# ztlpn/minilp

Hardware: AMD Instinct MI355X
Metric: simplex pivots/sec (higher is better)
Workload: dtype f64; 1 GPU; config 4: random LP 100000 vars x 100000 constraints, 100 nnz/row (0.1% fill), Max c'x, Ax<=b, x>=0; primal simplex with PSE+DSE from the slack basis; timed pivots 5..1983; parallelism=1 GPU, nucleus_size_at_end=1559, completed_steps=1978

## Files before the change

minilp_amd/csrc/engine.h:

```cpp
#pragma once
#include <hip/hip_runtime.h>

#include <cstdint>
#include <utility>
#include <stdexcept>
#include <string>
#include <vector>

#include "kernels.h"

namespace mlp {

enum Stage { STAGE_FTRAN = 0, STAGE_RATIO = 1, STAGE_BTRAN = 2, STAGE_BASIS = 3, STAGE_ROW = 4, STAGE_APPLY = 5 };

struct MlpError : std::runtime_error {
    int code;
    MlpError(int c, const std::string& s) : std::runtime_error(s), code(c) {}
};
struct LpFail {
    int code;
};

#define HIPCHECK(expr)                                                                                   \
    do {                                                                                                 \
// ... 285 lines not shown
    DevBuf<int> d_nb_order;
    DevBuf<int> d_pk_ptr;
    DevBuf<unsigned short> d_pk_row;
    DevBuf<double> d_pk_val;
    DevBuf<unsigned char> d_pk_valid;
    DevBuf<unsigned char> d_fmark;
    bool use_pack = true;
    bool pack_built = false;
    size_t band_total_ = 0;
    bool use_order = true;
    uint64_t order_built_at = 0;
    uint64_t lifetime_pivots = 0;
    uint64_t order_every = 2048;
    bool order_valid = false;
    uint64_t order_from = 4096;
    bool order_force = false;
    void refresh_nb_order(bool force);
    int det_mode = -1;
    int banded_mode = -1;
    bool use_banded() const;
  public:
    bool banded_active() const { return use_banded(); }
    bool factor_active() const { return fac_on_; }
    void restart_sampling() { batches_run = 0; }
  private:
    void ensure_banded();
    DevBuf<int> d_fpk_cnt, d_fpk_var;
    DevBuf<double> d_fpk_val, d_fpk_x, d_fpk_part;
    DevBuf<unsigned char> d_fpk_in;
    bool fpull_on_ = true;
    bool fpk_valid_ = false;
    uint64_t fpk_built_at_ = 0, fpk_builds_ = 0;
    int fpk_every_ = 1024;
    bool fpk_wanted() const;
    void fpk_rebuild();
    DevBuf<int> d_colblk;
    DevBuf<double> d_push_part;
    bool colblk_dirty = true;
    void ensure_colblk();
    DevBuf<double> d_sdiag_of_pos, d_W, d_U, d_V, d_Ut;
    int ld_pad = 16;
    int pad_for(int cap) const { return (cap >= 8192 || force_big_tiles) ? ld_pad : 0; }
    int ld() const { return cap_ + pad_for(cap_); }
    int lr_force = -1;
    DevBuf<double> d_work;
    DevBuf<double> d_alpha_r, d_helper;
    DevBuf<int2> d_nb_rng;
    int sweep_variant = 0;
    int sw_balanced = 1;
    int rt_device = 0;
    void acquire_runtime();
    void release_runtime();
    bool force_big_tiles = false;
    int shard_rank = 0, shard_world = 1;
    bool shard_defer_ = true;
    bool shard_live_ = false;
    bool shard_is_live() const { return shard_world > 1 && shard_live_; }
    MailRec* d_mail = nullptr;
    void* mail_host = nullptr;
    bool mail_registered = false;
    void* own_box = nullptr;
    void* peer_box[MAX_WORLD] = {};
    int mail_fanout = 1;
    size_t xb_cap_ = 0;
    bool no_wshard = false;
    void release_mailboxes();
    int pump_backend_ = 0;
// ... 106 lines not shown
```

minilp_amd/csrc/engine.hip:

```cpp
#include "engine.h"


#include <algorithm>
#include <chrono>
#include <cmath>
#include <cstdio>
#include <cstdlib>
#include <climits>
#include <cstring>
#include <limits>
#include <map>
#include <memory>
#include <mutex>

#include <dlfcn.h>
#include <fcntl.h>
#include <sys/mman.h>
#include <sys/stat.h>
#include <unistd.h>

namespace mlp {

static const double INF = std::numeric_limits<double>::infinity();
static double now_s() {
// ... 49 lines not shown
    force_big_tiles = bt && std::atoi(bt) != 0;
    const char* dm = std::getenv("MLP_DETERMINISTIC");
    if (dm) det_mode = std::atoi(dm) != 0 ? 1 : 0;
    const char* bd = std::getenv("MLP_BANDED");
    if (bd) banded_mode = std::atoi(bd) != 0 ? 1 : 0;
    const char* fr = std::getenv("MLP_FINAL_REFRESH");
    if (fr) final_refresh_pivots = std::atol(fr);
    if (const char* sp = std::getenv("MLP_SWEEP_PACKED")) use_pack = sp[0] != '0';
    if (const char* of = std::getenv("MLP_ORDER_FROM")) order_from = (uint64_t)std::atoll(of);
    if (const char* oe = std::getenv("MLP_ORDER_EVERY")) order_every = (uint64_t)std::atoll(oe);
    const char* lz = std::getenv("MLP_LAZY_DSE");
    lazy_dse = !(lz && lz[0] == '0');
    ratio_two = std::getenv("MLP_RATIO_TWO_KERNELS") != nullptr;
    if (const char* hy = std::getenv("MLP_HYPER")) hyper_mode = std::atoi(hy) > 0 ? 1 : 0;
    if (const char* phk = std::getenv("MLP_PRIMAL_HEAD_K")) ph_kmax = std::max(0, std::atoi(phk));
    if (const char* sbk = std::getenv("MLP_SMALL_BASIS_K")) sb_kmax = std::max(0, std::min(256, std::atoi(sbk)));
    if (const char* sk = std::getenv("MLP_STR_K")) str_kmax = std::atoi(sk);
    if (const char* hh = std::getenv("MLP_HYPER_HEAVY")) hyper_heavy = std::atol(hh);
    if (const char* rs = std::getenv("MLP_RATIO_SPIN_LIMIT")) ratio_spin_limit = std::atoll(rs);
    if (const char* sb = std::getenv("MLP_STREAM_BALANCED")) sw_balanced = std::atoi(sb);
    if (const char* fm = std::getenv("MLP_FACTOR")) fac_mode = std::atoi(fm) > 0 ? 1 : 0;
    if (const char* fj = std::getenv("MLP_FACTOR_J")) {
        fac_J_ = fac_period_ = std::max(1, std::min(64, std::atoi(fj)));
        fac_period_auto_ = false;
    }
    if (const char* ff = std::getenv("MLP_FACTOR_FROM")) fac_auto_cap_ = std::max(256, std::atoi(ff));
    if (const char* fb = std::getenv("MLP_FACTOR_BUMP")) {
        const int want = std::atoi(fb);
        fac_bump_max_ = std::max(0, std::min(FAC_BMAX, want));
        if (want < FAC_BMAX) fac_sb_max_ = std::min(fac_sb_max_, fac_bump_max_);
    }
    if (const char* fb = std::getenv("MLP_FACTOR_SB")) fac_sb_max_ = std::max(0, std::min(FAC_SB_MAX, std::atoi(fb)));
    if (const char* fb = std::getenv("MLP_FACTOR_SB_FROM")) fac_sb_from_ = std::max(1, std::atoi(fb));
    if (const char* fp = std::getenv("MLP_FPULL")) fpull_on_ = fp[0] != '0';
    const char* nws = std::getenv("MLP_NO_WSHARD");
    no_wshard = nws && std::atoi(nws) != 0;
    const char* bs = std::getenv("MLP_BATCH");
    if (bs) batch = std::max(1, std::min(RING, std::atoi(bs)));
    const char* gi = std::getenv("MLP_GRAPH_ITERS");
    if (gi) graph_iters = std::max(1, std::min(32, std::atoi(gi)));
}
namespace {
struct RtBundle {
    int device = 0;
    hipStream_t st = nullptr, st2 = nullptr;
    hipEvent_t evFork[3] = {nullptr, nullptr, nullptr}, evJoin[3] = {nullptr, nullptr, nullptr};
    Ctl* h_ctl = nullptr;
};
struct RtPool {
    std::mutex mu;
    std::vector<RtBundle> idle;
};
RtPool& rt_pool() {
    static RtPool* p = new RtPool();
    return *p;
}
constexpr size_t kMaxIdleRuntimes = 64;
}
void Engine::acquire_runtime() {
    int dev = 0;
    HIPCHECK(hipGetDevice(&dev));
    rt_device = dev;
    {
        RtPool& p = rt_pool();
        std::lock_guard<std::mutex> lk(p.mu);
        for (size_t i = 0; i < p.idle.size(); ++i)
            if (p.idle[i].device == dev) {
// ... 224 lines not shown
                d_pk_row.ensure(band_total_ + 16, 0, st);
                d_pk_val.ensure(band_total_ + 16, 0, st);
                if (d_pk_row.p != r0) HIPCHECK(hipMemsetAsync(d_pk_row.p, 0, sizeof(unsigned short) * d_pk_row.cap, st));
                if (d_pk_val.p != v0) HIPCHECK(hipMemsetAsync(d_pk_val.p, 0, sizeof(double) * d_pk_val.cap, st));
            }
            d_pk_valid.ensure((size_t)num_vars, 0, st);
            d_scan_tmp.ensure(np / 4096 + 8, 0, st);
        } catch (MlpError&) {
            (void)hipGetLastError();
            use_pack = false;
            return;
        }
        DevView t{};
        t.m = m_; t.n = num_vars; t.nbands = nb;
        t.bptr = d_bptr.p; t.brow = d_brow.p; t.bval = d_bval.p;
        t.nb_vars = d_nb_vars.p; t.nb_order = d_nb_order.p;
        launch_pack_count(t, d_pk_ptr.p, st);
        launch_exclusive_scan(d_pk_ptr.p, d_pk_ptr.p, (long)np, d_scan_tmp.p, st);
        launch_pack_fill(t, d_pk_ptr.p, d_pk_row.p, d_pk_val.p, d_pk_valid.p, st);
        HIPCHECK(hipStreamSynchronize(st));
        pack_built = true;
    }
}

void Engine::ensure_colblk() {
    if (!colblk_dirty) return;
    const int rb = (m_ + PB_ROWS - 1) / PB_ROWS;
    d_colblk.ensure((size_t)N_ * (rb + 1), 0, st);
    launch_build_colblk(d_cptr.p, d_crow.p, N_, rb, d_colblk.p, st);
    d_push_part.ensure((size_t)PB_CHUNKS * (size_t)m_, 0, st);
    colblk_dirty = false;
}

bool Engine::fpk_wanted() const {
    const int lr = fac_on_ ? 0 : (lr_force >= 0 ? lr_force : (cap_ >= 8192 ? 32 : 0));
    return fpull_on_ && !fac_on_ && !stepping && lr > 0 && enable_pse && d_rowinfo.p != nullptr;
}
void Engine::fpk_rebuild() {
    const size_t nnz = h_rcol.size();
    d_fpk_cnt.ensure((size_t)m_ + 8, 0, st);
    d_fpk_var.ensure(nnz + 8, 0, st);
    d_fpk_val.ensure(nnz + 8, 0, st);
    d_fpk_in.ensure((size_t)N_ + 8, 0, st);
    d_fpk_x.ensure((size_t)N_ + 8, 0, st);
    d_fpk_part.ensure(2 * (((size_t)m_ * 2 + 2048) / 32 + 8), 0, st);
    DevView t = *sync_view();
    t.fpk_cnt = d_fpk_cnt.p; t.fpk_var = d_fpk_var.p; t.fpk_val = d_fpk_val.p; t.fpk_in = d_fpk_in.p; t.fpk_x = d_fpk_x.p;
    HIPCHECK(hipMemsetAsync(d_fpk_in.p, 0, (size_t)N_, st));
    HIPCHECK(hipMemsetAsync(d_fpk_x.p, 0, sizeof(double) * (size_t)N_, st));
    launch_fpk_build(t, st);
    fpk_valid_ = true;
    fpk_built_at_ = lifetime_pivots;
    fpk_builds_ += 1;
    if (!hview.fpk_on || hview.fpk_cnt != d_fpk_cnt.p || hview.fpk_var != d_fpk_var.p || hview.fpk_val != d_fpk_val.p ||
        hview.fpk_in != d_fpk_in.p || hview.fpk_x != d_fpk_x.p || hview.fpk_part != d_fpk_part.p) {
        view_dirty = true;
        sync_view();
    }
}

DevView* Engine::sync_view() {
    if (!view_dirty) return &hview;
    DevView old = hview;
    DevView& v = hview;
    v.m = m_; v.n = num_vars; v.ld = ld(); v.pad0 = 0;
    v.csc_ptr = d_cptr.p; v.csc_row = d_crow.p; v.csc_val = d_cval.p;
    v.csr_ptr = d_rptr.p; v.csr_col = d_rcol.p; v.csr_val = d_rval.p;
    v.var_lo = d_lo.p; v.var_hi = d_hi.p; v.obj_c = d_obj.p;
    v.var_loc = d_var_loc.p;
    v.basic_vars = d_basic_vars.p; v.xB = d_xB.p; v.loB = d_loB.p; v.hiB = d_hiB.p; v.beta = d_beta.p;
    v.nb_vars = d_nb_vars.p; v.d = d_d.p; v.xN = d_xN.p; v.gamma = d_gamma.p; v.nbflags = d_nbflags.p;
    v.kslot_of_pos = d_kslot_of_pos.p; v.srow_of_pos = d_srow_of_pos.p; v.sdiag_of_pos = d_sdiag_of_pos.p;
    v.kslot_of_row = d_kslot_of_row.p; v.pos_of_srow = d_pos_of_srow.p; v.rowinfo = d_rowinfo.p;
    const bool shard_det = shard_world > 1;
    static const int pb_det_env = std::getenv("MLP_PB_DET") ? std::atoi(std::getenv("MLP_PB_DET")) : -1;
    int hbits = 1;
    while (hbits < 31 && (1 << hbits) <= max_row_nnz_) hbits += 1;
    const bool det_fits = hbits <= 20;
    const bool pb_det = det_fits && (shard_det || force_det_push_ || pb_det_env == 1 || (pb_det_env < 0 && pb_det_default));
    const bool pb_size = cap_ > 4096 || force_big_tiles ||
                         (shard_det && pb_det && cap_ >= 512 && det_mode != 1 && h_rcol.size() > ((size_t)1 << 21));
    v.pb_on = (pb_size && (!shard_det || pb_det)) ? 1 : 0;
    v.pb_det = (v.pb_on && pb_det) ? 1 : 0;
    v.pb_hbits = hbits;
    v.pb_amax = amax_;
    if (v.pb_on) ensure_colblk();
    v.colblk = v.pb_on ? d_colblk.p : nullptr;
    v.push_part = v.pb_on ? d_push_part.p : nullptr;
    v.pb_rb = (m_ + PB_ROWS - 1) / PB_ROWS;
    {
        if (!(fpk_wanted() && v.pb_on && (!v.pb_det || shard_world > 1))) fpk_valid_ = false;
        const bool fp = fpk_valid_ && d_fpk_cnt.p != nullptr;
        v.fpk_cnt = d_fpk_cnt.p; v.fpk_var = d_fpk_var.p; v.fpk_val = d_fpk_val.p; v.fpk_in = d_fpk_in.p;
        v.fpk_x = fp ? d_fpk_x.p : nullptr; v.fpk_part = d_fpk_part.p;
        v.fpk_on = fp ? 1 : 0; v.pad5 = 0;
    }
    v.det_pull = (!v.pb_on && (det_mode == 1 || shard_det || force_det_push_ || (det_mode < 0 && h_rcol.size() <= ((size_t)1 << 21)))) ? 1 : 0;
    if (v.det_pull) {
        const unsigned char* before = d_fmark.p;
        d_fmark.ensure((size_t)m_ + 64, 0, st);
        if (d_fmark.p != before) HIPCHECK(hipMemsetAsync(d_fmark.p, 0, d_fmark.cap, st));
        v.fmark = d_fmark.p;
    } else {
        v.fmark = nullptr;
    }
    v.banded = use_banded() ? 1 : 0;
    if (v.banded) ensure_banded();
    v.bptr = v.banded ? d_bptr.p : nullptr;
    v.brow = v.banded ? d_brow.p : nullptr;
    v.bval = v.banded ? d_bval.p : nullptr;
    v.band_part = v.banded ? d_band_part.p : nullptr;
    v.nbands = (m_ + BAND_ROWS - 1) / BAND_ROWS;
    if (v.banded && use_order && shard_world == 1 && (lifetime_pivots >= order_from || order_force)) {
        if (!order_valid || (use_pack && !pack_built)) refresh_nb_order(true);
        v.nb_order = d_nb_order.p;
    } else {
        v.nb_order = nullptr;
    }
    const bool pk = v.nb_order && use_pack && pack_built;
    v.pk_ptr = pk ? d_pk_ptr.p : nullptr; v.pk_row = pk ? d_pk_row.p : nullptr; v.pk_val = pk ? d_pk_val.p : nullptr;
    v.pk_valid = pk ? d_pk_valid.p : nullptr;
    v.pos_of_kslot = d_pos_of_kslot.p; v.row_of_kslot = d_row_of_kslot.p; v.W = d_W.p;
    v.U = d_U.p; v.V = d_V.p; v.Ut = d_Ut.p;
    v.lrJ = fac_on_ ? 0 : (lr_force >= 0 ? lr_force : (cap_ >= 8192 ? 32 : 0));
// ... 798 lines not shown
}
void Engine::get_values(double* out, int n) {
    fetch_values();
    for (int v = 0; v < n; ++v) {
        int loc = h_var_loc[v];
        out[v] = loc >= 0 ? h_xB[loc] : h_xN[-1 - loc];
    }
}
double Engine::cur_obj_val() {
    pull_ctl();
    return h_ctl->it.obj;
}

static const int kStageOrder[2][6] = {{STAGE_FTRAN, STAGE_RATIO, STAGE_BTRAN, STAGE_BASIS, STAGE_ROW, STAGE_APPLY},
                                      {STAGE_BTRAN, STAGE_ROW, STAGE_RATIO, STAGE_FTRAN, STAGE_BASIS, STAGE_APPLY}};
void Engine::launch_stage(int phase, int stage, bool with_events) {
    const DevView& dv = hview;
    const Geom g = geom();
    const int pse = enable_pse ? 1 : 0;
    const bool lazy = lazy_now(phase);
    const int dse = (enable_dse && !lazy) ? 1 : 0;
    const int wtau = lazy ? 0 : 1;
    const int inl = (dv.banded && phase == 0 && !stepping && !g.str) ? 1 : 0;
    if (dv.fac_on) {
        launch_stage_fac(phase, stage, with_events);
        return;
    }
    const bool phead = phase == 0 && pse && lazy && !stepping && shard_world == 1 && primal_head_supported(dv, g);
    const bool smallb = !phead && phase == 0 && pse && lazy && !stepping && !shard_is_live() && small_basis_supported(dv, g);
    const bool tkr = phase == 0 && pse && lazy && !stepping && shard_world == 1 && !smallb && !g.head_fused && !dv.pb_det && tk_rides_ratio(dv, g);
    const bool tkr_s = smallb && tk_rides_ratio_small(dv, g);
    const bool rkr = tkr && rk_rides_post(dv, g);
    const bool fpl_base = g.fp && phase == 0 && pse && lazy && !stepping && !smallb && !g.head_fused && max_col_nnz_ <= HEAD_LIST_CAP && fpull_supported(dv, g);
    const bool fpl = fpl_base && ((tkr && ftran_head_rides_gather(dv, g)) || (shard_world > 1 && dv.lrJ > 0 && dv.pb_on && !dv.det_pull && dv.rowinfo != nullptr));
    if (stage == STAGE_BASIS) touch_done = false;
    switch (stage) {
    case STAGE_FTRAN:
        if (with_events) HIPCHECK(hipEventRecord(ev[6], st));
        if (phead) {
            if (with_events) arm_kernel_timing(2, ev[2], ev[3]);
            launch_primal_head(dv, g, st);
            if (with_events) arm_kernel_timing(2, nullptr, nullptr);
            touch_done = true;
            if (with_events) HIPCHECK(hipEventRecord(ev[7], st));
            break;
        }
        if (phase == 0 && g.head_fused) {
            launch_ftran_fused(dv, g, 1, st);
        } else if (phase == 0 && !stepping && max_col_nnz_ <= HEAD_LIST_CAP && (fpl || ftran_head_rides_gather(dv, g))) {
            launch_ftran_gather_lrh(dv, g, st, tkr ? 1 : 0, fpl ? 1 : 0);
        } else {
            if (phase == 0) launch_ftran_prep(dv, 1, st);
            launch_ftran_gather(dv, g, st, tkr ? 1 : 0);
        }
        if (with_events && !fpl) HIPCHECK(hipEventRecord(ev[7], st));
        if (phase == 1) {
            launch_post_ftran(dv, g, pse, st);
            if (pse) launch_btran_rhs(dv, g, st);
        }
        break;
    case STAGE_RATIO:
        if (phead) break;
        if (fpl) {
            launch_fpull_ratio(dv, g, st, with_events ? ev[7] : nullptr);
        } else if (phase == 0) launch_ratio_primal(dv, g, pse, st, tkr ? 1 : (tkr_s ? 2 : 0));
        else launch_ratio_dual(dv, g, st, ar_built_ ? 1 : 0);
        break;
    case STAGE_BTRAN:
        if (phead || smallb || rkr) break;
        if (phase == 1 && g.head_fused) {
            launch_btran_fused(dv, g, 0, 1, st);
        } else {
            if (phase == 1) launch_btran_prep(dv, 1, 0, st);
            launch_btran(dv, g, (phase == 0 && !tkr && !fpl) ? pse : 0, st);
        }
        break;
    case STAGE_BASIS:
        if (phead) {
            touch_done = true;
            break;
        }
        if (smallb) {
            if (with_events) arm_kernel_timing(2, ev[2], ev[3]);
// ... 230 lines not shown
                stats.basis_changes += 1;
                if (r.kase >= 0 && r.kase < 5) stats.kase[r.kase] += 1;
                if (trace) trace_log.push_back({r.phase, r.q, r.r, ev_, lv, r.pivot_coeff, r.obj});
            }
        } else {
            result = r.status;
        }
    }
    (void)phase;
    return result;
}

int Engine::run_loop(int phase) {
    if (phase == 1) ensure_beta();
    if (fac_on_) pull_ctl();
    str_clean = false;
    batch_lazy = lazy_now(phase);
    bool fpk_fresh = false;
    for (;;) {
        if (pivot_budget == 0) {
            budget_exhausted = true;
            return ITER_PIVOT;
        }
        const bool long_run = use_graph && graph_iters > 1 && graph_batches_in_geom >= 8;
        const bool sample = profile && (sample_every == 1 || batches_run % (long_run ? 4 : 8) == 0);
        batches_run += 1;
        if (!hview.nb_order && use_order && lifetime_pivots >= order_from) view_dirty = true;
        sync_view();
        if (hview.nb_order) refresh_nb_order(false);
        if (hview.nb_order && use_pack && pack_built != (hview.pk_ptr != nullptr)) {
            view_dirty = true;
            sync_view();
        }
        if (phase == 0 && fpk_wanted() && hview.pb_on && (!hview.pb_det || shard_world > 1) && (!fpk_fresh || !fpk_valid_ || lifetime_pivots - fpk_built_at_ >= (uint64_t)fpk_every_)) {
            fpk_rebuild();
            fpk_fresh = true;
        }
        int hyper_gap = 0;
        if (hyper_off_until > lifetime_pivots && hyper_capable(phase))
            hyper_gap = (int)std::min<uint64_t>(hyper_off_until - lifetime_pivots, (uint64_t)1 << 20);
        if (!sample && hyper_gap == 0 && hyper_capable(phase)) {
            int B = RING;
            if (pivot_budget > 0 && (int64_t)B > pivot_budget) B = (int)pivot_budget;
            ensure_nucleus_cap(k_ + B + 1);
            if (fac_on_) continue;
            ensure_hyper();
            sync_view();
            launch_reset_ring(hview, st);
            launch_clear_work(hview, st);
            launch_hyper_dual(hview, enable_dse ? 1 : 0, B, hyper_heavy, st);
            str_clean = false;
            pull_ctl();
            const uint64_t before = stats.iterations;
            int res = process_records(phase, B);
            stats.hyper_iters += stats.iterations - before;
            if (h_ctl->hyper_bail) {
                stats.hyper_bails += 1;
                if (h_ctl->hyper_bail > 0 && h_ctl->hyper_bail < 10) stats.hyper_bail_reason[h_ctl->hyper_bail] += 1;
                if (stats.iterations - before >= 16) {
                    hyper_bail_streak = 0;
                    hyper_off_until = lifetime_pivots + 1;
                } else {
                    hyper_bail_streak = std::min(hyper_bail_streak + 1, hyper_backoff_max);
                    hyper_off_until = lifetime_pivots + ((uint64_t)2 << hyper_bail_streak);
                }
            } else if (stats.iterations - before >= 16) {
                hyper_bail_streak = 0;
// ... 1514 lines not shown
                if (!(bt[i] > 0.0) || !std::isfinite(bt[i])) throw MlpError(-1, "load_basis: non-positive or non-finite dual edge weight in the blob");
        }
        d_gamma.upload(gm, st); d_beta.upload(bt, st);
        HIPCHECK(hipStreamSynchronize(st));
        recalc_basic_vals();
        primal_feasible = basic_values_feasible();
        enable_pse = (h.flags & 4u) != 0;
        recalc_obj_coeffs();
        dual_feasible = reduced_costs_feasible();
        if (!primal_feasible && !dual_feasible)
            throw MlpError(-1, "load_basis: the basis is neither primal nor dual feasible for this model (the artificial-"
                               "objective phase needs a mode-2 checkpoint)");
        resume_in_optimize = primal_feasible && !dual_feasible;
    }
    iters_since_recalc = 0;
    iters_since_polish = 0;
    values_dirty = true;
    budget_exhausted = false;
    beta_stale = false;
    HIPCHECK(hipStreamSynchronize(st));
}

Engine* Engine::clone() {
    flush_lowrank();
    pull_maps();
    std::unique_ptr<Engine> owner(new Engine());
    Engine* e = owner.get();
    e->num_vars = num_vars; e->direction = direction;
    e->m_ = m_; e->N_ = N_;
    e->h_obj = h_obj; e->h_lo = h_lo; e->h_hi = h_hi; e->h_rhs = h_rhs;
    e->h_cons_row = h_cons_row;
    e->h_rptr = h_rptr; e->h_rcol = h_rcol; e->h_rval = h_rval;
    e->h_colnnz = h_colnnz; e->h_single_row = h_single_row; e->h_single_val = h_single_val;
    e->max_col_nnz_ = max_col_nnz_; e->max_row_nnz_ = max_row_nnz_; e->amax_ = amax_; e->fpull_on_ = fpull_on_;
    e->sw_balanced = sw_balanced; e->str_kmax = str_kmax; e->sb_kmax = sb_kmax; e->ph_kmax = ph_kmax; e->hyper_mode = hyper_mode; e->hyper_heavy = hyper_heavy; e->hyper_backoff_max = hyper_backoff_max; e->ratio_two = ratio_two; e->ratio_spin_limit = ratio_spin_limit; e->ranks_share_device = false; e->lazy_dse = lazy_dse; e->beta_stale = beta_stale; e->use_order = use_order; e->use_pack = use_pack; e->order_force = order_force; e->lifetime_pivots = lifetime_pivots;
    e->h_basic_vars = h_basic_vars; e->h_nb_vars = h_nb_vars; e->h_var_loc = h_var_loc;
    e->h_kslot_of_pos = h_kslot_of_pos; e->h_srow_of_pos = h_srow_of_pos; e->h_kslot_of_row = h_kslot_of_row;
    e->h_pos_of_srow = h_pos_of_srow; e->h_sdiag_of_pos = h_sdiag_of_pos; e->h_nb_fixed = h_nb_fixed;
    e->h_pos_of_kslot = h_pos_of_kslot; e->h_row_of_kslot = h_row_of_kslot;
    e->enable_pse = enable_pse; e->enable_dse = enable_dse;
    e->primal_feasible = primal_feasible; e->dual_feasible = dual_feasible;
    e->resume_in_optimize = resume_in_optimize;
    e->nnz_nonbasic = nnz_nonbasic;
    e->trace = trace; e->profile = profile;
    e->banded_mode = banded_mode; e->det_mode = det_mode;
    e->final_refresh_pivots = final_refresh_pivots; e->iters_since_recalc = iters_since_recalc;
    e->iters_since_polish = iters_since_polish;
    e->ld_pad = ld_pad; e->lr_force = lr_force; e->force_big_tiles = force_big_tiles;
    hipStream_t s2 = e->st;
    {
        const size_t nz = h_rcol.size();
        e->d_cptr.copy_from(d_cptr, (size_t)N_ + 1, s2); e->d_crow.copy_from(d_crow, nz, s2); e->d_cval.copy_from(d_cval, nz, s2);
        e->d_rptr.copy_from(d_rptr, (size_t)m_ + 1, s2); e->d_rcol.copy_from(d_rcol, nz, s2); e->d_rval.copy_from(d_rval, nz, s2);
        e->d_lo.copy_from(d_lo, (size_t)N_, s2); e->d_hi.copy_from(d_hi, (size_t)N_, s2); e->d_obj.copy_from(d_obj, (size_t)N_, s2);
        e->colblk_dirty = true;
        e->banded_dirty = true;
        e->view_dirty = true;
    }
    int mk = m_;
    e->m_ = 0;
    e->alloc_row_buffers(mk);
    e->m_ = mk;
    size_t mm = (size_t)m_, nn = (size_t)num_vars;
    e->d_var_loc.copy_from(d_var_loc, (size_t)N_, s2);
    e->d_basic_vars.copy_from(d_basic_vars, mm, s2);
    e->d_xB.copy_from(d_xB, mm, s2); e->d_loB.copy_from(d_loB, mm, s2); e->d_hiB.copy_from(d_hiB, mm, s2);
    e->d_beta.copy_from(d_beta, mm, s2);
// ... 50 lines not shown
    else if (w == "col_coeffs") from_dev_d(d_work.p, mm);
    else if (w == "row_coeffs") from_dev_d(d_alpha_r.p, nn);
    else if (w == "tau") from_dev_d(d_work.p + mm, mm);
    else if (w == "inv_basis_row_coeffs" || w == "v") {
        std::vector<double> both(2 * mm);
        if (mm) HIPCHECK(hipMemcpy(both.data(), d_work.p + 2 * mm, 2 * mm * sizeof(double), hipMemcpyDeviceToHost));
        tmp.resize(mm);
        const size_t off = (w == "v") ? 1 : 0;
        for (size_t i = 0; i < mm; ++i) tmp[i] = both[2 * i + off];
    } else if (w == "sq_norms_update_helper") from_dev_d(d_helper.p, nn);
    else if (w == "nb_flags") {
        std::vector<uint8_t> t(nn);
        if (nn) HIPCHECK(hipMemcpy(t.data(), d_nbflags.p, nn, hipMemcpyDeviceToHost));
        tmp.assign(t.begin(), t.end());
    } else if (w == "cur_obj_val") tmp = {cur_obj_val()};
    else if (w == "orig_obj_coeffs") tmp = h_obj;
    else if (w == "orig_var_mins") tmp = h_lo;
    else if (w == "orig_var_maxs") tmp = h_hi;
    else if (w == "orig_rhs") tmp = h_rhs;
    else if (w == "csr_indptr") tmp.assign(h_rptr.begin(), h_rptr.end());
    else if (w == "csr_indices") tmp.assign(h_rcol.begin(), h_rcol.end());
    else if (w == "csr_data") tmp = h_rval;
    else if (w == "flags") tmp = {(double)primal_feasible, (double)dual_feasible, (double)enable_pse, (double)enable_dse};
    else if (w == "small_basis_launches") {
        pull_ctl();
        tmp = {(double)h_ctl->sb_count};
    } else if (w == "dual_list_tests") {
        int n_ = 0, p_ = 0;
        HIPCHECK(hipMemcpy(&n_, &d_ctl.p->ar_used, sizeof(int), hipMemcpyDeviceToHost));
        HIPCHECK(hipMemcpy(&p_, &d_ctl.p->ar_pauses, sizeof(int), hipMemcpyDeviceToHost));
        tmp = {(double)n_, (double)p_};
    } else if (w == "fpull") {
        tmp = {(double)(hview.fpk_on ? 1 : 0), (double)fpk_builds_, (double)fpk_built_at_, (double)(fpull_supported(hview, geom()) ? 1 : 0)};
    } else if (w == "ratio_primal_form") {
        tmp = {(double)ratio_primal_form(hview, geom())};
    } else if (w == "golive_checks") {
        tmp = {(double)golive_checks_};
    } else if (w == "shard_live") {
        tmp = {(double)(shard_is_live() ? 1 : 0)};
    } else if (w == "primal_head_launches") {
        pull_ctl();
        tmp = {(double)h_ctl->ph_count};
    }
    else if (w == "hyper_profile") {
        pull_ctl();
        for (int i = 0; i < 13; ++i) tmp.push_back((double)h_ctl->hy_prof[i] * 0.01);
        tmp.push_back((double)h_ctl->hy_prof[13]);
        tmp.push_back((double)h_ctl->hy_prof[14] * 0.01);
        tmp.push_back(0.0);
        for (int i = 16; i < 24; ++i) tmp.push_back((double)h_ctl->hy_prof[i] * 0.01);
    }
    else if (w == "kernel_timeline") {
        pull_ctl();
        unsigned long long t0 = ~0ull;
        for (int i = 0; i < 24; ++i) if (h_ctl->hy_prof[i] && h_ctl->hy_prof[i] < t0) t0 = h_ctl->hy_prof[i];
        for (int i = 0; i < 24; ++i) tmp.push_back(h_ctl->hy_prof[i] ? (double)(h_ctl->hy_prof[i] - t0) * 0.01 : -1.0);
    }
    else if (w == "factor_plan") {
        if (fac_on_ && d_fac_meta.p && d_fac_segs.p) {
            int meta[8] = {0};
            HIPCHECK(hipStreamSynchronize(st));
            HIPCHECK(hipMemcpy(meta, d_fac_meta.p, sizeof(meta), hipMemcpyDeviceToHost));
            const int nseg = std::max(0, std::min(meta[7], FAC_MAX_LEVELS));
            std::vector<int> sg((size_t)3 * nseg), lp((size_t)meta[0] + 1);
            if (nseg) HIPCHECK(hipMemcpy(sg.data(), d_fac_segs.p, sizeof(int) * sg.size(), hipMemcpyDeviceToHost));
            HIPCHECK(hipMemcpy(lp.data(), d_fac_lptr.p, sizeof(int) * lp.size(), hipMemcpyDeviceToHost));
// ... 255 lines not shown
```

minilp_amd/csrc/kernels.h:

```cpp
#pragma once
#include <hip/hip_runtime.h>
#include <stdint.h>

namespace mlp {

constexpr double EPS = 1e-8;

enum IterStatus : int {
    ITER_PIVOT = 0,
    ITER_FLIP = 1,
    ITER_OPTIMAL = 2,
    ITER_UNBOUNDED = 3,
    ITER_FEASIBLE = 4,
    ITER_INFEASIBLE = 5,
    ITER_SINGULAR = 6,
    ITER_NONE = 7,
    ITER_COMM = 8,
    ITER_STALL = 9,
};

struct IterState {
    int status;
    int q;
    int r;
// ... 262 lines not shown
constexpr int TK_STRIDE = 1024;
constexpr int TK_WORDS = TK_STRIDE * (TK_GROUPS + 1) + 8;
constexpr int FAC_BAR_FLAG = TK_WORDS + 1024;

constexpr int FW_TR = 8;
constexpr int FW_TC = 1024;

constexpr int BAND_ROWS = 8192;
constexpr int BAND_THREADS = 1024;
constexpr int PB_ROWS = 4096;
constexpr int PB_CHUNKS = 48;
constexpr int PB_CHUNKS_DEFAULT = 24;

struct Geom {
    int m, n, cap;
    int lanes;
    int sweep_one;
    int sweep_variant;
    int big;
    int head_fused;
    int str;
    int sb;
    int fac;
    int ph;
    int ratio_two;
    int fp;
};

void launch_clear_work(const DevView& dv, hipStream_t st);
void launch_price_primal(const DevView& dv, const Geom& g, int use_pse, hipStream_t st);
void launch_price_dual(const DevView& dv, const Geom& g, int use_dse, hipStream_t st);
void launch_ftran_prep(const DevView& dv, int derive_primal, hipStream_t st);
void launch_ftran_gather(const DevView& dv, const Geom& g, hipStream_t st, int ys = 0);
void launch_ftran_fused(const DevView& dv, const Geom& g, int derive_primal, hipStream_t st);
bool ftran_head_rides_gather(const DevView& dv, const Geom& g);
void launch_ftran_gather_lrh(const DevView& dv, const Geom& g, hipStream_t st, int ys = 0, int fpk = 0);
bool fpull_supported(const DevView& dv, const Geom& g);
void launch_fpull_ratio(const DevView& dv, const Geom& g, hipStream_t st, hipEvent_t ftran_done = nullptr);
void launch_fpk_build(const DevView& dv, hipStream_t st);
void launch_btran_fused(const DevView& dv, const Geom& g, int with_rhs, int derive_dual, hipStream_t st);
constexpr int HEAD_LIST_CAP = 1024;
void launch_ratio_primal(const DevView& dv, const Geom& g, int use_pse, hipStream_t st, int tk_ride = 0);
bool tk_rides_ratio(const DevView& dv, const Geom& g);
int ratio_primal_form(const DevView& dv, const Geom& g);
bool tk_rides_ratio_small(const DevView& dv, const Geom& g);
void launch_post_ftran(const DevView& dv, const Geom& g, int use_pse, hipStream_t st);
void launch_btran_prep(const DevView& dv, int derive_dual, int plan_after, hipStream_t st);
void launch_btran(const DevView& dv, const Geom& g, int with_rhs, hipStream_t st, int after_fold = 0);
void launch_btran_rhs(const DevView& dv, const Geom& g, hipStream_t st);
bool launch_sweep(const DevView& dv, const Geom& g, int mode, int with_struct, hipStream_t st, int inline_combine = 0, int list = 0);
void launch_row_sparse(const DevView& dv, const Geom& g, int mode, int with_struct, int touch, hipStream_t st);
bool small_basis_supported(const DevView& dv, const Geom& g);
void launch_small_basis(const DevView& dv, const Geom& g, hipStream_t st, int tk_inside = 1);
bool primal_head_supported(const DevView& dv, const Geom& g);
int primal_head_kmax(int longest_column);
void launch_primal_head(const DevView& dv, const Geom& g, hipStream_t st);
void launch_init_nb_rng(const DevView& dv, const Geom& g, hipStream_t st);
void launch_ratio_dual(const DevView& dv, const Geom& g, hipStream_t st, int list_ok = 0);
void launch_fused_w(const DevView& dv, const Geom& g, int with_v, hipStream_t st, int with_tau = 1);
int launch_post_fused(const DevView& dv, const Geom& g, int with_v, hipStream_t st, int classic = 0, int skip_push = 0, int with_tau = 1, int touch = 0, int rk_ride = 0);
bool rk_rides_post(const DevView& dv, const Geom& g);
void launch_exact_beta(const DevView& dv, hipStream_t st);
void launch_hyper_dual(const DevView& dv, int use_dse, int max_iters, long heavy, hipStream_t st);
void launch_mail_handshake(const DevView& dv, int* out, hipStream_t st);
constexpr int MAIL_PUMP_RECS = MAIL_KINDS * 2 + 1;
void launch_mail_stage(const DevView& dv, void* stage, hipStream_t st);
void launch_mail_deliver(const DevView& dv, const void* stage, hipStream_t st);
// ... 100 lines not shown
```

minilp_amd/csrc/kernels.hip:

```cpp
#include "kernels.h"
#include <hip/hip_ext.h>

#include <limits.h>
#include <math.h>

#include <cstdlib>
#include <string>

namespace mlp {

#define NONE_IDX INT_MAX
constexpr int BLK = 256;

struct Cand {
    double key;
    int idx;
};
__device__ __forceinline__ Cand cand_none() { return Cand{-INFINITY, NONE_IDX}; }
__device__ __forceinline__ bool cand_better(const Cand& a, const Cand& b) {
    return a.key > b.key || (a.key == b.key && a.idx < b.idx);
}
__device__ __forceinline__ Cand wave_best(Cand c) {
#pragma unroll
    for (int o = 32; o > 0; o >>= 1) {
// ... 1702 lines not shown
    if (threadIdx.x == 0) {
        int r = c->it.r;
        if (v.kslot_of_pos[r] < 0) {
            double inv = 1.0 / v.sdiag_of_pos[r];
            sq += inv * inv;
        }
        c->it.rho_sq = sq;
    }
}
template <int G>
__global__ void __launch_bounds__(BLK) k_btran(DevView v, int n_gather, int after_fold = 0) {
    Ctl* c = v.ctl;
    if (c->halt || c->it.status != ITER_PIVOT) return;
    KMARK0(c, 7);
    const int k = c->k;
    if ((int)blockIdx.x < n_gather) {
        btran_rk_body(v, c, (int)blockIdx.x, n_gather, after_fold);
    } else {
        int slot = (((int)blockIdx.x - n_gather) * BLK + threadIdx.x) / G;
        int gl = threadIdx.x & (G - 1);
        if (slot >= k) return;
        int p = v.pos_of_kslot[slot];
        int var = v.basic_vars[p];
        int end = v.csc_ptr[var + 1];
        double acc = 0.0;
        for (int e = v.csc_ptr[var] + gl; e < end; e += G) acc += v.csc_val[e] * v.rv[v.csc_row[e]].y;
        acc = group_sum<G>(acc);
        if (gl == 0) v.tK[slot] = v.alpha_q[p] - acc;
    }
}


constexpr int HEAD_CAP = 1024;
__device__ void ftran_head_lds(const DevView& v, Ctl* c, int lane, int derive_primal, bool primary, int* ls, double* la, int* ln) {
    IterState* it = &c->it;
    const int q = it->q;
    const int var = v.nb_vars[q];
    if (primary && lane == 0) {
        it->entering_var = var;
        if (derive_primal) {
            double dq = v.d[q];
            it->sign = dq < 0.0;
            it->entering_cur = v.xN[q];
            it->entering_other = (dq < 0.0) ? v.var_hi[var] : v.var_lo[var];
            it->r = -1;
            it->leaving_var = -1;
        }
    }
    const bool atomic_land = !v.pb_on && !v.det_pull;
    const int base = v.csc_ptr[var], end = v.csc_ptr[var + 1];
    int cnt = 0;
    for (int e0 = base; e0 < end; e0 += 64) {
        const int e = e0 + lane;
        const bool valid = e < end;
        int s = -1;
        double a = 0.0;
        if (valid) {
            const int i = v.csc_row[e];
            a = v.csc_val[e];
            s = v.kslot_of_row[i];
            if (s < 0 && primary) {
                const int p = v.pos_of_srow[i];
                const double x = a / v.sdiag_of_pos[p];
                if (atomic_land) unsafeAtomicAdd(&v.alpha_q[p], x);
                else v.alpha_q[p] = x;
                if (aq_listing(v)) aq_list_add(v, c, p);
            }
        }
        const bool isk = valid && s >= 0;
        const unsigned long long mask = __ballot(isk);
        if (isk) {
            const int off = cnt + __popcll(mask & ((1ull << lane) - 1ull));
            if (off < HEAD_CAP) {
                ls[off] = s;
                la[off] = a;
            }
            if (primary) {
                v.klist_s[off] = s;
                v.klist_a[off] = a;
            }
        }
        cnt += __popcll(mask);
    }
    if (lane == 0) {
        *ln = cnt < HEAD_CAP ? cnt : HEAD_CAP;
        if (primary) it->klist_n = cnt;
    }
}
__global__ void __launch_bounds__(BLK) k_ftran_gather_lrh(DevView v, int fpk) {
    Ctl* c = v.ctl;
    if (c->halt || c->it.status != ITER_PIVOT) {
        if (blockIdx.x == 0 && threadIdx.x == 0) c->side_go = 0;
        return;
    }
    KMARK0(c, 0);
    __shared__ int s_ls[HEAD_CAP];
    __shared__ double s_la[HEAD_CAP];
    __shared__ double s_lrc[LR_MAX];
    __shared__ int s_n;
// ... 84 lines not shown
        int si[4];
#pragma unroll
        for (int u = 0; u < 4; ++u) {
            const int j = j0 + 4 * u;
            a[u] = j < n ? s_la[j] : 0.0;
            si[u] = j < n ? s_ls[j] : 0;
        }
#pragma unroll
        for (int u = 0; u < 4; ++u) w[u] = j0 + 4 * u < n ? wrow[si[u]] : 0.0;
#pragma unroll
        for (int u = 0; u < 4; ++u)
            if (j0 + 4 * u < n) acc += a[u] * w[u];
    }
    {
        double e[LR_MAX / 4], x[LR_MAX / 4];
#pragma unroll
        for (int u = 0; u < LR_MAX / 4; ++u) {
            const int j = gl + 4 * u;
            e[u] = j < nlow ? s_lrc[j] : 0.0;
            x[u] = j < nlow ? v.U[(size_t)j * v.ld + slot] : 0.0;
        }
#pragma unroll
        for (int u = 0; u < LR_MAX / 4; ++u)
            if (gl + 4 * u < nlow) acc += x[u] * e[u];
    }
    acc = group_sum<4>(acc);
    if (gl == 0) {
        v.aK[slot] = acc;
        v.alpha_q[p] = acc;
        if (fpk) v.fpk_x[fvar] = acc;
    }
}
template <int G>
__global__ void __launch_bounds__(BLK) k_ftran_fused(DevView v, int derive_primal) {
    Ctl* c = v.ctl;
    if (c->halt || c->it.status != ITER_PIVOT) return;
    KMARK0(c, 0);
    __shared__ int s_ls[HEAD_CAP];
    __shared__ double s_la[HEAD_CAP];
    __shared__ int s_n;
    if (threadIdx.x < 64) ftran_head_lds(v, c, threadIdx.x, derive_primal, blockIdx.x == 0, s_ls, s_la, &s_n);
    __syncthreads();
    const int slot = (blockIdx.x * BLK + threadIdx.x) / G;
    const int gl = threadIdx.x & (G - 1);
    if (slot >= c->k) return;
    const int n = s_n;
    double acc = 0.0;
    const double* wrow = v.W + (size_t)slot * v.ld;
    for (int j = gl; j < n; j += G) acc += s_la[j] * wrow[s_ls[j]];
    acc = group_sum<G>(acc);
    const int p = v.pos_of_kslot[slot];
    if (gl == 0) {
        v.aK[slot] = acc;
        v.alpha_q[p] = acc;
        if (acc != 0.0 && aq_listing(v)) aq_list_add(v, c, p);
    }
    if (acc != 0.0 && !v.pb_on && !v.det_pull) push_F<G>(v, p, acc, v.alpha_q, gl, aq_listing(v) ? c : nullptr);
    else if (acc != 0.0 && v.det_pull && v.fmark) mark_F<G>(v, p, gl);
}
__device__ void btran_head_lds(const DevView& v, Ctl* c, int lane, int derive_dual, bool primary, int* ls, double* la, int* ln) {
    IterState* it = &c->it;
    const int r = it->r;
    if (derive_dual && !c->forced && primary && lane == 0) {
        const double val = v.xB[r], mn = v.loB[r];
        it->leaving_new_val = (val < mn) ? mn : v.hiB[r];
        it->leaving_var = v.basic_vars[r];
        it->q = -1;
        it->entering_var = -1;
    }
    const int sr = v.kslot_of_pos[r];
    if (sr >= 0) {
        if (lane == 0) {
            ls[0] = sr;
            la[0] = 1.0;
            *ln = 1;
            if (primary) {
                v.blist_s[0] = sr;
                v.blist_a[0] = 1.0;
                it->blist_n = 1;
            }
        }
        return;
    }
    const int i_r = v.srow_of_pos[r];
// ... 2286 lines not shown
#include "primal_head.inc"
#include "factor.inc"
#include "factor_sb.inc"
#include "inverse.inc"

#define LANES_SWITCH(L, STMT4, STMT16, STMT32) \
    do {                                        \
        if ((L) <= 4) { STMT4; }                \
        else if ((L) <= 16) { STMT16; }         \
        else { STMT32; }                        \
    } while (0)

void launch_hyper_dual(const DevView& dv, int use_dse, int max_iters, long heavy, hipStream_t st) {
    const int prof_on = std::getenv("MLP_HYPER_PROF") != nullptr ? 1 : 0;
    static bool attr_set = false;
    if (!attr_set) {
        (void)hipFuncSetAttribute(reinterpret_cast<const void*>(k_hyper_dual), hipFuncAttributeMaxDynamicSharedMemorySize, (int)HY_LDS_BYTES);
        attr_set = true;
    }
    hipLaunchKernelGGL(k_hyper_dual, dim3(1), dim3(HB), HY_LDS_BYTES, st, dv, use_dse, max_iters, heavy > 0 ? heavy : HY_HEAVY, prof_on);
}
void launch_clear_work(const DevView& hv, hipStream_t st) {
    (void)hipMemsetAsync(hv.alpha_q, 0, sizeof(double) * 5 * (size_t)hv.m, st);
}
void launch_price_primal(const DevView& dv, const Geom& g, int use_pse, hipStream_t st) {
    hipLaunchKernelGGL(k_price_primal, dim3(grid_for(dv.nb_hi - dv.nb_lo)), dim3(BLK), 0, st, dv, use_pse);
}
void launch_price_dual(const DevView& dv, const Geom& g, int use_dse, hipStream_t st) {
    hipLaunchKernelGGL(k_price_dual, dim3(grid_for(g.m)), dim3(BLK), 0, st, dv, use_dse);
}
void launch_ftran_prep(const DevView& dv, int derive_primal, hipStream_t st) {
    hipLaunchKernelGGL(k_ftran_prep, dim3(1), dim3(64), 0, st, dv, derive_primal);
}
void launch_ftran_fused(const DevView& dv, const Geom& g, int derive_primal, hipStream_t st) {
    LANES_SWITCH(g.lanes,
                 hipLaunchKernelGGL(k_ftran_fused<4>, dim3(blocks_for((long)g.cap * 4)), dim3(BLK), 0, st, dv, derive_primal),
                 hipLaunchKernelGGL(k_ftran_fused<16>, dim3(blocks_for((long)g.cap * 16)), dim3(BLK), 0, st, dv, derive_primal),
                 hipLaunchKernelGGL(k_ftran_fused<64>, dim3(blocks_for((long)g.cap * 64)), dim3(BLK), 0, st, dv, derive_primal));
    if (dv.pb_on) launch_blocked_push(dv, 0, st);
    else if (dv.det_pull) launch_pull_F(dv, g, 0, st);
}
void launch_btran_fused(const DevView& dv, const Geom& g, int with_rhs, int derive_dual, hipStream_t st) {
    int n_gather = blocks_for(g.cap);
    if (n_gather > 512) n_gather = 512;
#define BTRANF(G)                                                                                                  \
    do {                                                                                                           \
        int n_rhs = with_rhs ? blocks_for((long)g.cap * G) : 0;                                                    \
        hipLaunchKernelGGL(k_btran_fused<G>, dim3(n_gather + n_rhs), dim3(BLK), 0, st, dv, n_gather, derive_dual); \
    } while (0)
    LANES_SWITCH(g.lanes, BTRANF(4), BTRANF(16), BTRANF(64));
#undef BTRANF
}
bool ftran_head_rides_gather(const DevView& dv, const Geom& g) {
    return dv.lrJ > 0 && dv.pb_on && dv.world <= 1 && !g.fac && !dv.det_pull && dv.rowinfo != nullptr;
}
void launch_ftran_gather_lrh(const DevView& dv, const Geom& g, hipStream_t st, int ys, int fpk) {
    hipLaunchKernelGGL(k_ftran_gather_lrh, dim3(blocks_for((long)g.cap * 4)), dim3(BLK), 0, st, dv, fpk);
    if (!fpk) launch_blocked_push(dv, 0, st, ys);
}
void launch_ftran_gather(const DevView& dv, const Geom& g, hipStream_t st, int ys) {
    LANES_SWITCH((dv.lrJ && dv.pb_on) ? 4 : g.lanes,
                 hipLaunchKernelGGL(k_ftran_gather<4>, dim3(blocks_for((long)g.cap * 4)), dim3(BLK), 0, st, dv),
                 hipLaunchKernelGGL(k_ftran_gather<16>, dim3(blocks_for((long)g.cap * 16)), dim3(BLK), 0, st, dv),
                 hipLaunchKernelGGL(k_ftran_gather<64>, dim3(blocks_for((long)g.cap * 64)), dim3(BLK), 0, st, dv));
    if (dv.pb_on) launch_blocked_push(dv, 0, st, ys);
    else if (dv.det_pull) launch_pull_F(dv, g, 0, st);
}
static int coresident_half(const void* fn, int slot) {
    static int cache[3][64];
    static bool known[3][64];
    int dev = 0;
// ... 2 lines not shown
        int per_cu = 0, cus = 0;
        if (hipOccupancyMaxActiveBlocksPerMultiprocessor(&per_cu, fn, BLK, 0) == hipSuccess &&
            hipDeviceGetAttribute(&cus, hipDeviceAttributeMultiprocessorCount, dev) == hipSuccess)
            cache[slot][dev] = per_cu * cus / 2;
        else
            cache[slot][dev] = 0;
        known[slot][dev] = true;
    }
    return cache[slot][dev];
}
static bool ratio_one_enabled() {
    const char* e = std::getenv("MLP_RATIO_ONE");
    return !(e && e[0] == '0');
}
bool tk_rides_ratio(const DevView& dv, const Geom& g) {
    const char* e = std::getenv("MLP_TK_RIDE");
    if (e && e[0] == '0') return false;
    if (dv.world > 1 || !dv.pb_on || !dv.lrJ || g.ratio_two || g.cap <= 0) return false;
    if (g.m <= 16384 && ratio_one_enabled()) return false;
    const int nb = grid_for(g.m);
    const int max_coresident = coresident_half(reinterpret_cast<const void*>(k_ratio_primal_fused), 0);
    return nb <= max_coresident && (long)nb * BLK * 4 >= (long)g.m;
}
bool tk_rides_ratio_small(const DevView& dv, const Geom& g) {
    const char* e = std::getenv("MLP_TK_RIDE");
    if (e && e[0] == '0') return false;
    if (dv.world > 1 || g.ratio_two || g.cap <= 0 || !dv.rowinfo) return false;
    if (g.m <= 16384 && ratio_one_enabled()) return false;
    const int nb = grid_for(g.m);
    const int max_coresident = coresident_half(reinterpret_cast<const void*>(k_ratio_primal_fused), 0);
    return nb <= max_coresident && (long)nb * BLK * 4 >= (long)g.m;
}
bool fpull_supported(const DevView& dv, const Geom& g) {
    return dv.fpk_on && dv.fpk_cnt && dv.rowinfo && dv.lrJ > 0 && (long)grid_for(g.m) * BLK * 4 >= (long)g.m;
}
void launch_fpull_ratio(const DevView& dv, const Geom& g, hipStream_t st, hipEvent_t ftran_done) {
    const long items = (long)g.m + (long)g.cap;
    const int n1 = blocks_for(items * FP_G);
    hipLaunchKernelGGL(k_fpull_p1, dim3(n1), dim3(BLK), 0, st, dv);
    if (ftran_done) (void)hipEventRecord(ftran_done, st);
    const int nb = grid_for(g.m);
    const int lanes = g.lanes <= 4 ? 4 : (g.lanes <= 16 ? 16 : 64);
    LANES_SWITCH(lanes, hipLaunchKernelGGL(k_fpull_p2<4>, dim3(nb + blocks_for((long)g.cap * 4) + 1), dim3(BLK), 0, st, dv, nb, n1),
                 hipLaunchKernelGGL(k_fpull_p2<16>, dim3(nb + blocks_for((long)g.cap * 16) + 1), dim3(BLK), 0, st, dv, nb, n1),
                 hipLaunchKernelGGL(k_fpull_p2<64>, dim3(nb + blocks_for((long)g.cap * 64) + 1), dim3(BLK), 0, st, dv, nb, n1));
}
int ratio_primal_form(const DevView& dv, const Geom& g) {
    if (dv.world <= 1 && g.m <= 16384 && ratio_one_enabled()) return 0;
    const int nb = grid_for(g.m);
    const int max_coresident = g.ratio_two ? 0 : coresident_half(reinterpret_cast<const void*>(k_ratio_primal_fused), 0);
    return (nb <= max_coresident && (long)nb * BLK * 4 >= (long)g.m) ? 1 : 2;
}
void launch_ratio_primal(const DevView& dv, const Geom& g, int use_pse, hipStream_t st, int tk_ride) {
    if (tk_ride) {
        const int nb = grid_for(g.m);
        const int lanes = g.lanes <= 4 ? 4 : (g.lanes <= 16 ? 16 : 64);
        hipLaunchKernelGGL(k_ratio_primal_fused, dim3(nb + blocks_for((long)g.cap * lanes)), dim3(BLK), 0, st, dv, tk_ride == 2 ? use_pse : 2, nb, lanes,
                           tk_ride == 2 ? 1 : 0);
        return;
    }
    const int form = ratio_primal_form(dv, g);
    if (form == 0) {
        hipLaunchKernelGGL(k_ratio_primal_one, dim3(1), dim3(BLK), 0, st, dv, use_pse);
        return;
    }
    const int nb = grid_for(g.m);
    if (form == 1) {
// ... 426 lines not shown
```

Measured before the change: 10640 pivots/s.

## Extend fused pull-based FTRAN ratio path to head-fused non-blocked configuration

Adds a second mode for the pull-based ratio path (fpk) that applies when FTRAN uses the fused head kernel without blocked push or low-rank J. In this mode the fused FTRAN kernel writes each basic variable's value into the fpk_x scatter array and skips the atomic landing, list building and the blocked push or pull-F step. The subsequent fpull ratio kernels then compute the column from the row-packed structure. This is meant to avoid the scatter/push cost for the mid-size configuration. The change enlarges the partial buffer, relaxes fpull_supported to drop the lrJ requirement, and adds an MLP_FPK_EVERY override.

After: 10220 pivots/s. -3.9%, worse.

```diff
diff --git a/minilp_amd/csrc/engine.h b/minilp_amd/csrc/engine.h
--- a/minilp_amd/csrc/engine.h
+++ b/minilp_amd/csrc/engine.h
@@ -341,7 +341,9 @@
     bool fpk_valid_ = false;
     uint64_t fpk_built_at_ = 0, fpk_builds_ = 0;
     int fpk_every_ = 1024;
-    bool fpk_wanted() const;
+    bool fpull_force_ = false;
+    int fpull_mode_ = 0;
+    bool fpk_serves(bool pb_on, bool pb_det) const;
     void fpk_rebuild();
     DevBuf<int> d_colblk;
     DevBuf<double> d_push_part;
diff --git a/minilp_amd/csrc/engine.hip b/minilp_amd/csrc/engine.hip
--- a/minilp_amd/csrc/engine.hip
+++ b/minilp_amd/csrc/engine.hip
@@ -105,7 +105,11 @@
     }
     if (const char* fb = std::getenv("MLP_FACTOR_SB")) fac_sb_max_ = std::max(0, std::min(FAC_SB_MAX, std::atoi(fb)));
     if (const char* fb = std::getenv("MLP_FACTOR_SB_FROM")) fac_sb_from_ = std::max(1, std::atoi(fb));
-    if (const char* fp = std::getenv("MLP_FPULL")) fpull_on_ = fp[0] != '0';
+    if (const char* fp = std::getenv("MLP_FPULL")) {
+        fpull_on_ = fp[0] != '0';
+        fpull_force_ = fp[0] == '2';
+    }
+    if (const char* fe = std::getenv("MLP_FPK_EVERY")) fpk_every_ = std::max(1, std::atoi(fe));
     const char* nws = std::getenv("MLP_NO_WSHARD");
     no_wshard = nws && std::atoi(nws) != 0;
     const char* bs = std::getenv("MLP_BATCH");
@@ -396,9 +400,12 @@
     colblk_dirty = false;
 }
 
-bool Engine::fpk_wanted() const {
-    const int lr = fac_on_ ? 0 : (lr_force >= 0 ? lr_force : (cap_ >= 8192 ? 32 : 0));
-    return fpull_on_ && !fac_on_ && !stepping && lr > 0 && enable_pse && d_rowinfo.p != nullptr;
+bool Engine::fpk_serves(bool pb_on, bool pb_det) const {
+    if (!fpull_on_ || fac_on_ || stepping || !enable_pse || d_rowinfo.p == nullptr) return false;
+    const int lr = lr_force >= 0 ? lr_force : (cap_ >= 8192 ? 32 : 0);
+    if (lr > 0) return pb_on && (!pb_det || shard_world > 1);
+    const bool det_pull = det_mode == 1 || (det_mode < 0 && h_rcol.size() <= ((size_t)1 << 21));
+    return shard_world == 1 && !pb_on && !str_now && (fpull_force_ || !det_pull) && max_col_nnz_ <= HEAD_LIST_CAP && max_row_nnz_ <= HEAD_LIST_CAP;
 }
 void Engine::fpk_rebuild() {
     const size_t nnz = h_rcol.size();
@@ -407,7 +414,7 @@
     d_fpk_val.ensure(nnz + 8, 0, st);
     d_fpk_in.ensure((size_t)N_ + 8, 0, st);
     d_fpk_x.ensure((size_t)N_ + 8, 0, st);
-    d_fpk_part.ensure(2 * (((size_t)m_ * 2 + 2048) / 32 + 8), 0, st);
+    d_fpk_part.ensure(2 * (((size_t)m_ * 3 + 8192) / 32 + 8), 0, st);
     DevView t = *sync_view();
     t.fpk_cnt = d_fpk_cnt.p; t.fpk_var = d_fpk_var.p; t.fpk_val = d_fpk_val.p; t.fpk_in = d_fpk_in.p; t.fpk_x = d_fpk_x.p;
     HIPCHECK(hipMemsetAsync(d_fpk_in.p, 0, (size_t)N_, st));
@@ -453,7 +460,7 @@
     v.push_part = v.pb_on ? d_push_part.p : nullptr;
     v.pb_rb = (m_ + PB_ROWS - 1) / PB_ROWS;
     {
-        if (!(fpk_wanted() && v.pb_on && (!v.pb_det || shard_world > 1))) fpk_valid_ = false;
+        if (!fpk_serves(v.pb_on != 0, v.pb_det != 0)) fpk_valid_ = false;
         const bool fp = fpk_valid_ && d_fpk_cnt.p != nullptr;
         v.fpk_cnt = d_fpk_cnt.p; v.fpk_var = d_fpk_var.p; v.fpk_val = d_fpk_val.p; v.fpk_in = d_fpk_in.p;
         v.fpk_x = fp ? d_fpk_x.p : nullptr; v.fpk_part = d_fpk_part.p;
@@ -1318,7 +1325,11 @@
     const bool tkr_s = smallb && tk_rides_ratio_small(dv, g);
     const bool rkr = tkr && rk_rides_post(dv, g);
     const bool fpl_base = g.fp && phase == 0 && pse && lazy && !stepping && !smallb && !g.head_fused && max_col_nnz_ <= HEAD_LIST_CAP && fpull_supported(dv, g);
-    const bool fpl = fpl_base && ((tkr && ftran_head_rides_gather(dv, g)) || (shard_world > 1 && dv.lrJ > 0 && dv.pb_on && !dv.det_pull && dv.rowinfo != nullptr));
+    const bool fpl_l = fpl_base && dv.lrJ > 0 && ((shard_world == 1 && !dv.pb_det && ratio_primal_form(dv, g) != 0 && ftran_head_rides_gather(dv, g)) || (shard_world > 1 && dv.pb_on && !dv.det_pull && dv.rowinfo != nullptr));
+    const bool fpl_m = g.fp && phase == 0 && pse && lazy && !stepping && !phead && !smallb && g.head_fused && !g.str && shard_world == 1 && !dv.pb_on && !dv.lrJ &&
+                       fpull_supported(dv, g);
+    const bool fpl = fpl_l || fpl_m;
+    if (stage == STAGE_RATIO && phase == 0) fpull_mode_ = fpl_m ? 2 : (fpl_l ? 1 : 0);
     if (stage == STAGE_BASIS) touch_done = false;
     switch (stage) {
     case STAGE_FTRAN:
@@ -1332,9 +1343,9 @@
             break;
         }
         if (phase == 0 && g.head_fused) {
-            launch_ftran_fused(dv, g, 1, st);
-        } else if (phase == 0 && !stepping && max_col_nnz_ <= HEAD_LIST_CAP && (fpl || ftran_head_rides_gather(dv, g))) {
-            launch_ftran_gather_lrh(dv, g, st, tkr ? 1 : 0, fpl ? 1 : 0);
+            launch_ftran_fused(dv, g, 1, st, fpl_m ? 1 : 0);
+        } else if (phase == 0 && !stepping && max_col_nnz_ <= HEAD_LIST_CAP && (fpl_l || ftran_head_rides_gather(dv, g))) {
+            launch_ftran_gather_lrh(dv, g, st, tkr ? 1 : 0, fpl_l ? 1 : 0);
         } else {
             if (phase == 0) launch_ftran_prep(dv, 1, st);
             launch_ftran_gather(dv, g, st, tkr ? 1 : 0);
@@ -1631,7 +1642,7 @@
             view_dirty = true;
             sync_view();
         }
-        if (phase == 0 && fpk_wanted() && hview.pb_on && (!hview.pb_det || shard_world > 1) && (!fpk_fresh || !fpk_valid_ || lifetime_pivots - fpk_built_at_ >= (uint64_t)fpk_every_)) {
+        if (phase == 0 && fpk_serves(hview.pb_on != 0, hview.pb_det != 0) && (!fpk_fresh || !fpk_valid_ || lifetime_pivots - fpk_built_at_ >= (uint64_t)fpk_every_)) {
             fpk_rebuild();
             fpk_fresh = true;
         }
@@ -3212,7 +3223,7 @@
     e->h_cons_row = h_cons_row;
     e->h_rptr = h_rptr; e->h_rcol = h_rcol; e->h_rval = h_rval;
     e->h_colnnz = h_colnnz; e->h_single_row = h_single_row; e->h_single_val = h_single_val;
-    e->max_col_nnz_ = max_col_nnz_; e->max_row_nnz_ = max_row_nnz_; e->amax_ = amax_; e->fpull_on_ = fpull_on_;
+    e->max_col_nnz_ = max_col_nnz_; e->max_row_nnz_ = max_row_nnz_; e->amax_ = amax_; e->fpull_on_ = fpull_on_; e->fpull_force_ = fpull_force_;
     e->sw_balanced = sw_balanced; e->str_kmax = str_kmax; e->sb_kmax = sb_kmax; e->ph_kmax = ph_kmax; e->hyper_mode = hyper_mode; e->hyper_heavy = hyper_heavy; e->hyper_backoff_max = hyper_backoff_max; e->ratio_two = ratio_two; e->ratio_spin_limit = ratio_spin_limit; e->ranks_share_device = false; e->lazy_dse = lazy_dse; e->beta_stale = beta_stale; e->use_order = use_order; e->use_pack = use_pack; e->order_force = order_force; e->lifetime_pivots = lifetime_pivots;
     e->h_basic_vars = h_basic_vars; e->h_nb_vars = h_nb_vars; e->h_var_loc = h_var_loc;
     e->h_kslot_of_pos = h_kslot_of_pos; e->h_srow_of_pos = h_srow_of_pos; e->h_kslot_of_row = h_kslot_of_row;
@@ -3329,6 +3340,13 @@
         tmp = {(double)n_, (double)p_};
     } else if (w == "fpull") {
         tmp = {(double)(hview.fpk_on ? 1 : 0), (double)fpk_builds_, (double)fpk_built_at_, (double)(fpull_supported(hview, geom()) ? 1 : 0)};
+    } else if (w == "fpull_mode") {
+        DevView t = hview;
+        t.fpk_on = 1;
+        if (!t.fpk_cnt) t.fpk_cnt = reinterpret_cast<int*>(d_ctl.p);
+        if (!t.fpk_x) t.fpk_x = reinterpret_cast<double*>(d_ctl.p);
+        if (!t.rowinfo) t.rowinfo = reinterpret_cast<RowInfo*>(d_ctl.p);
+        tmp = {(double)fpull_mode_, (double)(fpull_supported(t, geom()) ? 1 : 0)};
     } else if (w == "ratio_primal_form") {
         tmp = {(double)ratio_primal_form(hview, geom())};
     } else if (w == "golive_checks") {
diff --git a/minilp_amd/csrc/kernels.h b/minilp_amd/csrc/kernels.h
--- a/minilp_amd/csrc/kernels.h
+++ b/minilp_amd/csrc/kernels.h
@@ -318,7 +318,7 @@
 void launch_price_dual(const DevView& dv, const Geom& g, int use_dse, hipStream_t st);
 void launch_ftran_prep(const DevView& dv, int derive_primal, hipStream_t st);
 void launch_ftran_gather(const DevView& dv, const Geom& g, hipStream_t st, int ys = 0);
-void launch_ftran_fused(const DevView& dv, const Geom& g, int derive_primal, hipStream_t st);
+void launch_ftran_fused(const DevView& dv, const Geom& g, int derive_primal, hipStream_t st, int fpk = 0);
 bool ftran_head_rides_gather(const DevView& dv, const Geom& g);
 void launch_ftran_gather_lrh(const DevView& dv, const Geom& g, hipStream_t st, int ys = 0, int fpk = 0);
 bool fpull_supported(const DevView& dv, const Geom& g);
diff --git a/minilp_amd/csrc/kernels.hip b/minilp_amd/csrc/kernels.hip
--- a/minilp_amd/csrc/kernels.hip
+++ b/minilp_amd/csrc/kernels.hip
@@ -1758,7 +1758,7 @@
 
 
 constexpr int HEAD_CAP = 1024;
-__device__ void ftran_head_lds(const DevView& v, Ctl* c, int lane, int derive_primal, bool primary, int* ls, double* la, int* ln) {
+__device__ void ftran_head_lds(const DevView& v, Ctl* c, int lane, int derive_primal, bool primary, int* ls, double* la, int* ln, int fpk = 0) {
     IterState* it = &c->it;
     const int q = it->q;
     const int var = v.nb_vars[q];
@@ -1773,7 +1773,7 @@
             it->leaving_var = -1;
         }
     }
-    const bool atomic_land = !v.pb_on && !v.det_pull;
+    const bool atomic_land = !fpk && !v.pb_on && !v.det_pull;
     const int base = v.csc_ptr[var], end = v.csc_ptr[var + 1];
     int cnt = 0;
     for (int e0 = base; e0 < end; e0 += 64) {
@@ -1790,7 +1790,7 @@
                 const double x = a / v.sdiag_of_pos[p];
                 if (atomic_land) unsafeAtomicAdd(&v.alpha_q[p], x);
                 else v.alpha_q[p] = x;
-                if (aq_listing(v)) aq_list_add(v, c, p);
+                if (!fpk && aq_listing(v)) aq_list_add(v, c, p);
             }
         }
         const bool isk = valid && s >= 0;
@@ -1941,14 +1941,14 @@
     }
 }
 template <int G>
-__global__ void __launch_bounds__(BLK) k_ftran_fused(DevView v, int derive_primal) {
+__global__ void __launch_bounds__(BLK) k_ftran_fused(DevView v, int derive_primal, int fpk) {
     Ctl* c = v.ctl;
     if (c->halt || c->it.status != ITER_PIVOT) return;
     KMARK0(c, 0);
     __shared__ int s_ls[HEAD_CAP];
     __shared__ double s_la[HEAD_CAP];
     __shared__ int s_n;
-    if (threadIdx.x < 64) ftran_head_lds(v, c, threadIdx.x, derive_primal, blockIdx.x == 0, s_ls, s_la, &s_n);
+    if (threadIdx.x < 64) ftran_head_lds(v, c, threadIdx.x, derive_primal, blockIdx.x == 0, s_ls, s_la, &s_n, fpk);
     __syncthreads();
     const int slot = (blockIdx.x * BLK + threadIdx.x) / G;
     const int gl = threadIdx.x & (G - 1);
@@ -1956,9 +1956,18 @@
     const int n = s_n;
     double acc = 0.0;
     const double* wrow = v.W + (size_t)slot * v.ld;
+    const int p = v.pos_of_kslot[slot];
+    const int fvar = fpk ? v.basic_vars[p] : 0;
     for (int j = gl; j < n; j += G) acc += s_la[j] * wrow[s_ls[j]];
     acc = group_sum<G>(acc);
-    const int p = v.pos_of_kslot[slot];
+    if (fpk) {
+        if (gl == 0) {
+            v.aK[slot] = acc;
+            v.alpha_q[p] = acc;
+            v.fpk_x[fvar] = acc;
+        }
+        return;
+    }
     if (gl == 0) {
         v.aK[slot] = acc;
         v.alpha_q[p] = acc;
@@ -4311,11 +4320,12 @@
 void launch_ftran_prep(const DevView& dv, int derive_primal, hipStream_t st) {
     hipLaunchKernelGGL(k_ftran_prep, dim3(1), dim3(64), 0, st, dv, derive_primal);
 }
-void launch_ftran_fused(const DevView& dv, const Geom& g, int derive_primal, hipStream_t st) {
+void launch_ftran_fused(const DevView& dv, const Geom& g, int derive_primal, hipStream_t st, int fpk) {
     LANES_SWITCH(g.lanes,
-                 hipLaunchKernelGGL(k_ftran_fused<4>, dim3(blocks_for((long)g.cap * 4)), dim3(BLK), 0, st, dv, derive_primal),
-                 hipLaunchKernelGGL(k_ftran_fused<16>, dim3(blocks_for((long)g.cap * 16)), dim3(BLK), 0, st, dv, derive_primal),
-                 hipLaunchKernelGGL(k_ftran_fused<64>, dim3(blocks_for((long)g.cap * 64)), dim3(BLK), 0, st, dv, derive_primal));
+                 hipLaunchKernelGGL(k_ftran_fused<4>, dim3(blocks_for((long)g.cap * 4)), dim3(BLK), 0, st, dv, derive_primal, fpk),
+                 hipLaunchKernelGGL(k_ftran_fused<16>, dim3(blocks_for((long)g.cap * 16)), dim3(BLK), 0, st, dv, derive_primal, fpk),
+                 hipLaunchKernelGGL(k_ftran_fused<64>, dim3(blocks_for((long)g.cap * 64)), dim3(BLK), 0, st, dv, derive_primal, fpk));
+    if (fpk) return;
     if (dv.pb_on) launch_blocked_push(dv, 0, st);
     else if (dv.det_pull) launch_pull_F(dv, g, 0, st);
 }
@@ -4384,7 +4394,7 @@
     return nb <= max_coresident && (long)nb * BLK * 4 >= (long)g.m;
 }
 bool fpull_supported(const DevView& dv, const Geom& g) {
-    return dv.fpk_on && dv.fpk_cnt && dv.rowinfo && dv.lrJ > 0 && (long)grid_for(g.m) * BLK * 4 >= (long)g.m;
+    return dv.fpk_on && dv.fpk_cnt && dv.fpk_x && dv.rowinfo && (long)grid_for(g.m) * BLK * 4 >= (long)g.m;
 }
 void launch_fpull_ratio(const DevView& dv, const Geom& g, hipStream_t st, hipEvent_t ftran_done) {
     const long items = (long)g.m + (long)g.cap;
```
